# szy4017/DeepSense6G_TII

Hardware: AMD Instinct MI355X
Metric: training samples/sec (5-frame seq, bs=12 per GPU) (higher is better)
Workload: dtype f32; 1 GPU; BASELINE configs[2]: full camera+LiDAR+radar+GPS fusion, 5x(3+1+2)x256x256 + 2x2 GPS per sample, bs=12 per GPU, sigmoid focal loss, AdamW, train-mode BN, dropout 0.1; global_batch=12, seq_len=5, parallelism=dp1, ema=False, launch=eager, optimizer=AdamW after backward

## Files before the change

deepsense6g_tii_amd/csrc/igemm.hip:

```cpp
#include "common.h"
#include "gemm_plan.h"
#include <vector>

extern int g_ds6g_attn_fused128;
extern int g_ds6g_attn_merged_sum;
extern int g_ds6g_attn_percu;
extern int g_ds6g_attn_handover;
extern int g_wino_kb64;

#ifndef IGEMM_STAGES_FD
#define IGEMM_STAGES_FD 3
#endif
#ifndef IGEMM_STAGES_W
#define IGEMM_STAGES_W 2
#endif

GCLK_STORAGE(g_igemm_clk, g_igemm_wg, ds6g_igemm_clocks_read)

namespace {

enum { MODE_FWD = 0, MODE_DGRAD = 1, MODE_WGRAD = 2 };

struct IgemmParams {
    const float* a_src;
    const float* b_src;
    float* out;
    int N, H, W, C;
    int Ho, Wo, K;
    int R, S, stride, pad;
    int Mg, Ng, Kg;
    const float* bias;
    const float* residual;
    const float* mask_src;
    int relu;
    int accumulate;
    uint32_t drop_thr;
    float drop_scale;
    uint64_t seed;
    uint64_t seed_off;
    const uint64_t* salt;
    int k_per_split;
    size_t split_stride;
    int tiles_n;
    int nclass;
    double prof_flops;
    int wg_rows;
    int is_linear;
    int want_colsum;
    int xcd_splits;
    int h0, hstep, Hs, w0, wstep, Ws, r0, rstep, nr, s0, sstep, ns;
    unsigned a_bytes, b_bytes;
    int dbg;
};


template <int MODE, int BM, int BN, int EPI, int BK, int BF, int FAST>
__global__ __launch_bounds__(256) void igemm_kernel(const IgemmParams pin) {
    IgemmParams p = pin;
    if (EPI && p.drop_thr && p.salt) p.seed_off += *p.salt;
    GCLK_DECL(g_igemm_wg);
    if (MODE == MODE_DGRAD && pin.nclass > 1) {
        const int ph = blockIdx.y >> 1, pw = blockIdx.y & 1;
        p.h0 = ph;
        p.w0 = pw;
        p.r0 = (ph + p.pad) & 1;
        p.nr = p.r0 < p.R ? (p.R - p.r0 + 1) / 2 : 0;
        p.s0 = (pw + p.pad) & 1;
        p.ns = p.s0 < p.S ? (p.S - p.s0 + 1) / 2 : 0;
        p.Kg = p.nr * p.ns * p.K;
        if (p.ns == 0) p.ns = 1;
        if (p.Kg == 0 && p.accumulate) return;
    }
    constexpr int CH = BK / 4;
    constexpr int RPB = 16 / CH;
    constexpr int KH = BK / 2;
    constexpr int TM = BM / 64;
    constexpr int TN = BN / 64;
    constexpr int A_LD = BM * CH / 256;
    constexpr int B_LD = BN * CH / 256;
    constexpr bool A_KMAJOR = (MODE == MODE_WGRAD);
    constexpr bool B_KMAJOR = (MODE != MODE_FWD);
    __shared__ __attribute__((aligned(16))) float As0[BM * BK];
    __shared__ __attribute__((aligned(16))) float As1[BM * BK];
    __shared__ __attribute__((aligned(16))) float Bs0[BN * BK];
    __shared__ __attribute__((aligned(16))) float Bs1[BN * BK];
    constexpr int NS = (MODE == MODE_WGRAD) ? IGEMM_STAGES_W : (BK == 32 ? 2 : IGEMM_STAGES_FD);
    static_assert(NS >= 2 && NS <= 4, "2..4 LDS stages");
    __shared__ __attribute__((aligned(16))) float As2[NS >= 3 ? BM * BK : 4];
    __shared__ __attribute__((aligned(16))) float Bs2[NS >= 3 ? BN * BK : 4];
    __shared__ __attribute__((aligned(16))) float As3[NS >= 4 ? BM * BK : 4];
    __shared__ __attribute__((aligned(16))) float Bs3[NS >= 4 ? BN * BK : 4];

    const int tid = threadIdx.x;
    const int lane = tid & 63;
    const int wave = __builtin_amdgcn_readfirstlane(tid >> 6);
    const int wm = wave >> 1, wn = wave & 1;
    int wg, split = blockIdx.z;
    if (MODE == MODE_WGRAD && p.xcd_splits) {
        const int nwg = gridDim.x * gridDim.z, orig = blockIdx.x + gridDim.x * blockIdx.z;
        const int q = nwg >> 3, r = nwg & 7, xcd = orig & 7;
        const int lin = (xcd < r ? xcd * (q + 1) : r * (q + 1) + (xcd - r) * q) + (orig >> 3);
        split = lin / (int)gridDim.x;
        wg = lin - split * (int)gridDim.x;
    } else {
        const int nwg = gridDim.x, orig = blockIdx.x;
        const int q = nwg >> 3, r = nwg & 7, xcd = orig & 7;
        wg = (xcd < r ? xcd * (q + 1) : r * (q + 1) + (xcd - r) * q) + (orig >> 3);
    }
    const int tile_m = wg / p.tiles_n;
    const int tile_n = wg - tile_m * p.tiles_n;
    const int m0 = tile_m * BM, n0 = tile_n * BN;
    const int kbegin = (MODE == MODE_WGRAD) ? split * p.k_per_split : 0;
    const int kend = (MODE == MODE_WGRAD) ? min(p.Kg, kbegin + p.k_per_split) : p.Kg;
    const int nk = (kend - kbegin + BK - 1) / BK;

    const i32x4 a_rsrc = make_srd(p.a_src, p.a_bytes);
    const i32x4 b_rsrc = make_srd(p.b_src, p.b_bytes);

    unsigned a_base[A_LD];
    int a_y[A_LD], a_x[A_LD];
    int a_c[A_LD], a_r[A_LD], a_s[A_LD], a_k[A_LD];
    bool a_ok[A_LD];
#pragma unroll
    for (int i = 0; i < A_LD; ++i) {
        const int idx = tid + i * 256;
        if (MODE == MODE_FWD || MODE == MODE_DGRAD) {
            const int row = idx / CH;
            const int m = m0 + row;
            a_ok[i] = m < p.Mg;
            const int mm = a_ok[i] ? m : 0;
            const int cin = (MODE == MODE_FWD) ? p.C : p.K;
            const int kg = ((idx % CH) ^ ((row / RPB) & (CH - 1))) * 4;
            a_k[i] = kg;
            const int tap = kg / cin;
            a_c[i] = kg - tap * cin;
            const int nsx = (MODE == MODE_DGRAD) ? p.ns : p.S;
            a_r[i] = tap / nsx;
            a_s[i] = tap - a_r[i] * nsx;
            if (MODE == MODE_FWD) {
                int ow, t, oh, n;
                fast_divmod(mm, p.Wo, t, ow);
                fast_divmod(t, p.Ho, n, oh);
                a_y[i] = oh * p.stride - p.pad;
                a_x[i] = ow * p.stride - p.pad;
                a_base[i] = (unsigned)n * (unsigned)(p.H * p.W * p.C);
            } else {
                int ww, t, hh, n;
                fast_divmod(mm, p.Ws, t, ww);
                fast_divmod(t, p.Hs, n, hh);
                a_y[i] = p.h0 + hh * p.hstep + p.pad;
                a_x[i] = p.w0 + ww * p.wstep + p.pad;
                a_base[i] = (unsigned)n * (unsigned)(p.Ho * p.Wo * p.K);
            }
        } else {
            const int mc = idx % (BM / 4);
            a_ok[i] = (m0 + mc * 4) < p.Mg;
            a_k[i] = kbegin + idx / (BM / 4);
            a_base[i] = (unsigned)(m0 + mc * 4);
            a_y[i] = a_x[i] = a_c[i] = a_r[i] = a_s[i] = 0;
        }
    }
    unsigned b_base[B_LD];
    int b_r[B_LD], b_s[B_LD];
    int b_k[B_LD];
    int b_o[B_LD], b_t[B_LD];
    int b_n[B_LD];
    bool b_ok[B_LD];
#pragma unroll
    for (int i = 0; i < B_LD; ++i) {
        const int idx = tid + i * 256;
        b_r[i] = b_s[i] = b_o[i] = b_t[i] = b_n[i] = 0;
        if (MODE == MODE_FWD) {
            const int row = idx / CH;
            b_ok[i] = (n0 + row) < p.Ng;
            b_k[i] = ((idx % CH) ^ ((row / RPB) & (CH - 1))) * 4;
            b_base[i] = (unsigned)(n0 + row) * (unsigned)p.Kg;
        } else if (MODE == MODE_DGRAD) {
            b_ok[i] = (n0 + (idx % (BN / 4)) * 4) < p.Ng;
            const int kg = idx / (BN / 4);
            b_k[i] = kg;
            const int tap = kg / p.K;
            b_o[i] = kg - tap * p.K;
            b_t[i] = tap / p.ns;
            b_n[i] = tap - b_t[i] * p.ns;
            b_base[i] = (unsigned)(n0 + (idx % (BN / 4)) * 4);
        } else {
            const int ncol = n0 + (idx % (BN / 4)) * 4;
            b_ok[i] = ncol < p.Ng;
            const int nn = b_ok[i] ? ncol : 0;
            const int tap = nn / p.C;
            b_r[i] = tap / p.S;
            b_s[i] = tap - b_r[i] * p.S;
            b_base[i] = (unsigned)(nn - tap * p.C);
            const int pix = kbegin + idx / (BN / 4);
            b_k[i] = pix;
            const int pp = pix < p.Kg ? pix : 0;
            b_o[i] = pp % p.Wo;
            const int t = pp / p.Wo;
            b_t[i] = t % p.Ho;
            b_n[i] = t / p.Ho;
        }
    }

    [[maybe_unused]] int u_c0 = 0, u_r = 0, u_s = 0;
    [[maybe_unused]] unsigned u_kb = 0;
    [[maybe_unused]] int u_kpos = kbegin, u_n = 0, u_oh = 0, u_ow = 0;
    [[maybe_unused]] unsigned a_vo[A_LD], b_vo[B_LD];
    [[maybe_unused]] int a_kr[A_LD], b_kr[B_LD], b_ihl[B_LD], b_iwl[B_LD];
    [[maybe_unused]] i32x4 b_rsrc_f = b_rsrc;
    auto retap = [&]() {
#pragma unroll
        for (int i = 0; i < A_LD; ++i) {
            if (MODE == MODE_FWD) {
                const int ih = a_y[i] + u_r, iw = a_x[i] + u_s;
                const bool ok = a_ok[i] && (unsigned)ih < (unsigned)p.H && (unsigned)iw < (unsigned)p.W;
                a_vo[i] = ok ? (a_base[i] + (unsigned)((ih * p.W + iw) * p.C + a_c[i])) * 4u : OOB_OFF;
            } else if (MODE == MODE_DGRAD) {
                const int th = a_y[i] - (p.r0 + u_r * p.rstep), tw = a_x[i] - (p.s0 + u_s * p.sstep);
                int oh = th, ow = tw;
                bool okk = th >= 0 && tw >= 0;
                if (p.stride == 2) {
                    oh = th >> 1;
                    ow = tw >> 1;
                    okk = okk && !((th | tw) & 1);
                } else if (p.stride != 1) {
                    oh = th / p.stride;
                    ow = tw / p.stride;
                    okk = okk && (oh * p.stride == th) && (ow * p.stride == tw);
                }
                const bool ok = a_ok[i] && okk && oh < p.Ho && ow < p.Wo;
                a_vo[i] = ok ? (a_base[i] + (unsigned)((oh * p.Wo + ow) * p.K + a_c[i])) * 4u : OOB_OFF;
            }
        }
    };
    if (FAST) {
        if (MODE == MODE_FWD) {
            retap();
#pragma unroll
            for (int i = 0; i < B_LD; ++i) b_vo[i] = b_ok[i] ? (b_base[i] + (unsigned)b_k[i]) * 4u : OOB_OFF;
        } else if (MODE == MODE_DGRAD) {
            retap();
#pragma unroll
            for (int i = 0; i < B_LD; ++i)
                b_vo[i] = b_ok[i] ? (b_base[i] + (unsigned)(b_o[i] * (p.R * p.S) * p.C)) * 4u : OOB_OFF;
        } else {
            if (p.wg_rows == 0) {
                u_ow = kbegin % p.Wo;
                const int t = kbegin / p.Wo;
                u_oh = t % p.Ho;
                u_n = t / p.Ho;
            } else {
                const int t = kbegin / p.Wo;
                u_oh = t % p.Ho;
                u_n = t / p.Ho;
            }
            const int shift = (p.pad * p.W + p.pad) * p.C;
            b_rsrc_f = make_srd(p.b_src - shift, p.b_bytes + (unsigned)shift * 4u);
#pragma unroll
            for (int i = 0; i < A_LD; ++i) {
                a_kr[i] = (tid + i * 256) / (BM / 4);
                a_vo[i] = (a_base[i] + (unsigned)(a_kr[i] * p.K)) * 4u;
            }
#pragma unroll
            for (int i = 0; i < B_LD; ++i) {
                b_kr[i] = (tid + i * 256) / (BN / 4);
                const int dl_oh = p.wg_rows == 0 ? 0 : b_kr[i] / p.Wo;
                const int dl_ow = p.wg_rows == 0 ? b_kr[i] : b_kr[i] % p.Wo;
                b_ihl[i] = dl_oh * p.stride - p.pad + b_r[i];
                b_iwl[i] = dl_ow * p.stride - p.pad + b_s[i];
                b_vo[i] = (unsigned)((int)b_base[i] + (b_ihl[i] * p.W + b_iwl[i]) * p.C + shift) * 4u;
            }
        }
    }

    auto issue_tiles = [&](float* Ad, float* Bd) {
        if (FAST) {
            if (MODE == MODE_FWD || MODE == MODE_DGRAD) {
                const unsigned sa = (unsigned)u_c0 * 4u;
                unsigned sb;
                if (MODE == MODE_FWD) {
                    sb = u_kb;
                } else {
                    const int tapw = (p.r0 + u_r * p.rstep) * p.S + p.s0 + u_s * p.sstep;
                    sb = (unsigned)((u_c0 * (p.R * p.S) + tapw) * p.C) * 4u;
                }
#pragma unroll
                for (int i = 0; i < A_LD; ++i)
                    dma16(a_rsrc, lds_addr(Ad) + (unsigned)(i * 256 + wave * 64) * 16u, (p.dbg & 32) ? OOB_OFF : a_vo[i], sa);
#pragma unroll
                for (int i = 0; i < B_LD; ++i)
                    dma16(b_rsrc, lds_addr(Bd) + (unsigned)(i * 256 + wave * 64) * 16u, (p.dbg & 32) ? OOB_OFF : b_vo[i], sb);
                u_kb += BK * 4;
                u_c0 += BK;
                if (u_c0 == ((MODE == MODE_FWD) ? p.C : p.K)) {
                    u_c0 = 0;
                    if (++u_s == ((MODE == MODE_FWD) ? p.S : p.ns)) { u_s = 0; ++u_r; }
                    retap();
                }
            } else {
                const int rows_left = kend - u_kpos;
                const unsigned sa = (unsigned)(u_kpos * p.K) * 4u;
                const int ihu = u_oh * p.stride, iwu = u_ow * p.stride;
                const unsigned sb = (unsigned)(((u_n * p.H + ihu) * p.W + iwu) * p.C) * 4u;
#pragma unroll
                for (int i = 0; i < A_LD; ++i) {
                    const bool ok = a_ok[i] && a_kr[i] < rows_left && !(p.dbg & 32);
                    dma16(a_rsrc, lds_addr(Ad) + (unsigned)(i * 256 + wave * 64) * 16u, ok ? a_vo[i] : OOB_OFF, sa);
                }
#pragma unroll
                for (int i = 0; i < B_LD; ++i) {
                    const bool ok = b_ok[i] && b_kr[i] < rows_left && (unsigned)(ihu + b_ihl[i]) < (unsigned)p.H &&
                                    (unsigned)(iwu + b_iwl[i]) < (unsigned)p.W && !(p.dbg & 32);
                    dma16(b_rsrc_f, lds_addr(Bd) + (unsigned)(i * 256 + wave * 64) * 16u, ok ? b_vo[i] : OOB_OFF, sb);
                }
                u_kpos += BK;
                if (p.wg_rows == 0) {
                    u_ow += BK;
                    if (u_ow >= p.Wo) {
                        u_ow = 0;
                        if (++u_oh == p.Ho) { u_oh = 0; ++u_n; }
                    }
                } else {
                    u_oh += p.wg_rows;
                    if (u_oh >= p.Ho) { u_oh = 0; ++u_n; }
                }
            }
            return;
        }
#pragma unroll
        for (int i = 0; i < A_LD; ++i) {
            unsigned off;
            bool ok = a_ok[i] && a_k[i] < kend;
            if (MODE == MODE_FWD) {
                const int ih = a_y[i] + a_r[i], iw = a_x[i] + a_s[i];
                ok = ok && ih >= 0 && ih < p.H && iw >= 0 && iw < p.W;
                off = a_base[i] + (unsigned)((ih * p.W + iw) * p.C + a_c[i]);
            } else if (MODE == MODE_DGRAD) {
                const int th = a_y[i] - (p.r0 + a_r[i] * p.rstep), tw = a_x[i] - (p.s0 + a_s[i] * p.sstep);
                int oh = th, ow = tw;
                bool okk = th >= 0 && tw >= 0;
                if (p.stride == 2) {
                    oh = th >> 1;
                    ow = tw >> 1;
                    okk = okk && !((th | tw) & 1);
                } else if (p.stride != 1) {
                    oh = th / p.stride;
                    ow = tw / p.stride;
                    okk = okk && (oh * p.stride == th) && (ow * p.stride == tw);
                }
                ok = ok && okk && oh < p.Ho && ow < p.Wo;
                off = a_base[i] + (unsigned)((oh * p.Wo + ow) * p.K + a_c[i]);
            } else {
                off = a_base[i] + (unsigned)a_k[i] * (unsigned)p.K;
            }
            if (p.dbg & 32) ok = false;
            dma16(a_rsrc, lds_addr(Ad) + (unsigned)(i * 256 + wave * 64) * 16u, ok ? off * 4u : OOB_OFF, 0u);
            a_k[i] += BK;
            if (MODE != MODE_WGRAD) {
                const int cin = (MODE == MODE_FWD) ? p.C : p.K;
                a_c[i] += BK;
                const int nsx = (MODE == MODE_DGRAD) ? p.ns : p.S;
                while (a_c[i] >= cin) {
                    a_c[i] -= cin;
                    if (++a_s[i] == nsx) { a_s[i] = 0; ++a_r[i]; }
                }
            }
        }
#pragma unroll
        for (int i = 0; i < B_LD; ++i) {
            unsigned off;
            bool ok = b_ok[i] && b_k[i] < kend;
            if (MODE == MODE_FWD) {
                off = b_base[i] + (unsigned)b_k[i];
            } else if (MODE == MODE_DGRAD) {
                const int tap = (p.r0 + b_t[i] * p.rstep) * p.S + p.s0 + b_n[i] * p.sstep;
                off = b_base[i] + (unsigned)((b_o[i] * (p.R * p.S) + tap) * p.C);
                b_o[i] += BK;
                while (b_o[i] >= p.K) {
                    b_o[i] -= p.K;
                    if (++b_n[i] == p.ns) { b_n[i] = 0; ++b_t[i]; }
                }
            } else {
                const int ih = b_t[i] * p.stride - p.pad + b_r[i];
                const int iw = b_o[i] * p.stride - p.pad + b_s[i];
                ok = ok && ih >= 0 && ih < p.H && iw >= 0 && iw < p.W;
                off = b_base[i] + (unsigned)(((b_n[i] * p.H + ih) * p.W + iw) * p.C);
                b_o[i] += BK;
                while (b_o[i] >= p.Wo) {
                    b_o[i] -= p.Wo;
                    if (++b_t[i] == p.Ho) { b_t[i] = 0; ++b_n[i]; }
                }
            }
            if (p.dbg & 32) ok = false;
            dma16(b_rsrc, lds_addr(Bd) + (unsigned)(i * 256 + wave * 64) * 16u, ok ? off * 4u : OOB_OFF, 0u);
            b_k[i] += BK;
        }
    };

    f32x16 acc[TM][TN];
#pragma unroll
    for (int i = 0; i < TM; ++i)
#pragma unroll
        for (int j = 0; j < TN; ++j)
#pragma unroll
            for (int r = 0; r < 16; ++r) acc[i][j][r] = 0.f;

    const int a_row = wm * (BM / 2) + (lane & 31);
    const int b_row = wn * (BN / 2) + (lane & 31);
    const int khalf = lane >> 5;
    const int swz = ((lane & 31) / RPB) & (CH - 1);

    float csum = 0.f;
    const bool do_csum = (MODE == MODE_WGRAD) && p.want_colsum && tile_n == 0 && tid < BM;
    auto k_step = [&](const float* Ac, const float* Bc, float* An, float* Bn, int rem) {
        if (NS >= 3) {
            if (NS >= 4 && rem >= 2) asm volatile("s_waitcnt vmcnt(%0)" ::"n"(2 * (A_LD + B_LD)) : "memory");
            else if (rem >= 1) asm volatile("s_waitcnt vmcnt(%0)" ::"n"(A_LD + B_LD) : "memory");
            else asm volatile("s_waitcnt vmcnt(0)" ::: "memory");
            GCLK(g_igemm_clk, 4);
            if (!(p.dbg & 4)) __syncthreads();
            GCLK(g_igemm_clk, 5);
        }
        if (rem >= NS - 1 && !(p.dbg & 1)) issue_tiles(An, Bn);
        GCLK(g_igemm_clk, 2);
        if (MODE == MODE_WGRAD && do_csum) {
#pragma unroll
            for (int k = 0; k < BK; ++k) csum += Ac[k * BM + tid];
        }
        float af[TM][KH], bf[TN][KH];
#pragma unroll
        for (int i = 0; i < TM; ++i) {
            if (A_KMAJOR) {
#pragma unroll
                for (int kk = 0; kk < KH; ++kk) af[i][kk] = Ac[(khalf * KH + kk) * BM + a_row + i * 32];
            } else {
                const float* rp = &Ac[(a_row + i * 32) * BK];
#pragma unroll
                for (int c = 0; c < CH / 2; ++c) {
                    const f32x4 v = *reinterpret_cast<const f32x4*>(rp + (((khalf * (CH / 2) + c) ^ swz) << 2));
#pragma unroll
                    for (int e = 0; e < 4; ++e) af[i][4 * c + e] = v[e];
                }
            }
        }
#pragma unroll
        for (int j = 0; j < TN; ++j) {
            if (B_KMAJOR) {
#pragma unroll
                for (int kk = 0; kk < KH; ++kk) bf[j][kk] = Bc[(khalf * KH + kk) * BN + b_row + j * 32];
            } else {
                const float* rp = &Bc[(b_row + j * 32) * BK];
#pragma unroll
                for (int c = 0; c < CH / 2; ++c) {
                    const f32x4 v = *reinterpret_cast<const f32x4*>(rp + (((khalf * (CH / 2) + c) ^ swz) << 2));
#pragma unroll
                    for (int e = 0; e < 4; ++e) bf[j][4 * c + e] = v[e];
                }
            }
        }
        __builtin_amdgcn_sched_barrier(0);
        if (BF) {
            static_assert(!BF || BK % 16 == 0, "bf16 k-tiles are multiples of 16");
#pragma unroll
            for (int q = 0; q < BK / 16; ++q) {
                if (BF == 3) {
                    bf16x8 ah[TM], am[TM], al3[TM], bh[TN], bm[TN], bl3[TN];
#pragma unroll
                    for (int i = 0; i < TM; ++i) split3_bf16x8(&af[i][8 * q], ah[i], am[i], al3[i]);
#pragma unroll
                    for (int j = 0; j < TN; ++j) split3_bf16x8(&bf[j][8 * q], bh[j], bm[j], bl3[j]);
#pragma unroll
                    for (int i = 0; i < TM; ++i)
#pragma unroll
                        for (int j = 0; j < TN; ++j)
                            acc[i][j] = mfma_x6(ah[i], am[i], al3[i], bh[j], bm[j], bl3[j], acc[i][j]);
                    continue;
                }
                bf16x8 a8[TM], b8[TN], al[TM], bl[TN];
#pragma unroll
                for (int i = 0; i < TM; ++i) {
                    if (BF == 2) split_bf16x8(&af[i][8 * q], a8[i], al[i]);
                    else {
#pragma unroll
                        for (int e = 0; e < 8; ++e) a8[i][e] = (__bf16)af[i][8 * q + e];
                    }
                }
#pragma unroll
                for (int j = 0; j < TN; ++j) {
                    if (BF == 2) split_bf16x8(&bf[j][8 * q], b8[j], bl[j]);
                    else {
#pragma unroll
                        for (int e = 0; e < 8; ++e) b8[j][e] = (__bf16)bf[j][8 * q + e];
                    }
                }
                if (BF == 2) {
#pragma unroll
                    for (int i = 0; i < TM; ++i)
#pragma unroll
                        for (int j = 0; j < TN; ++j)
                            acc[i][j] = __builtin_amdgcn_mfma_f32_32x32x16_bf16(al[i], b8[j], acc[i][j], 0, 0, 0);
#pragma unroll
                    for (int i = 0; i < TM; ++i)
#pragma unroll
                        for (int j = 0; j < TN; ++j)
                            acc[i][j] = __builtin_amdgcn_mfma_f32_32x32x16_bf16(a8[i], bl[j], acc[i][j], 0, 0, 0);
                }
#pragma unroll
                for (int i = 0; i < TM; ++i)
#pragma unroll
                    for (int j = 0; j < TN; ++j)
                        acc[i][j] = __builtin_amdgcn_mfma_f32_32x32x16_bf16(a8[i], b8[j], acc[i][j], 0, 0, 0);
            }
        } else {
#pragma unroll
            for (int kk = 0; kk < BK / 2; ++kk) {
#pragma unroll
                for (int i = 0; i < TM; ++i)
#pragma unroll
                    for (int j = 0; j < TN; ++j)
                        acc[i][j] = __builtin_amdgcn_mfma_f32_32x32x2f32(af[i][kk], bf[j][kk], acc[i][j], 0, 0, 0);
            }
        }
        __builtin_amdgcn_sched_barrier(0);
        GCLK(g_igemm_clk, 3);
        GCLK_COUNT(g_igemm_clk, 15);
        if (NS == 2) {
            asm volatile("s_waitcnt vmcnt(0)" ::: "memory");
            GCLK(g_igemm_clk, 4);
            if (!(p.dbg & 4)) __syncthreads();
            GCLK(g_igemm_clk, 5);
        }
    };

    float* const Ast[4] = {As0, As1, As2, As3};
    float* const Bst[4] = {Bs0, Bs1, Bs2, Bs3};
    [[maybe_unused]] float bias_pre[TN];
    if (EPI) {
#pragma unroll
        for (int j = 0; j < TN; ++j) {
            const int col = n0 + wn * (BN / 2) + j * 32 + (lane & 31);
            bias_pre[j] = (p.bias && col < p.Ng) ? p.bias[col] : 0.f;
        }
    }
    GCLK(g_igemm_clk, 0);
#pragma unroll
    for (int u = 0; u < NS - 1; ++u)
        if (u < nk && !(p.dbg & 16)) issue_tiles(Ast[u], Bst[u]);
    if (NS == 2) {
        asm volatile("s_waitcnt vmcnt(0)" ::: "memory");
        __syncthreads();
    }
    GCLK(g_igemm_clk, 1);
    for (int kt0 = 0; kt0 < nk; kt0 += NS) {
#pragma unroll
        for (int u = 0; u < NS; ++u) {
            const int kt = kt0 + u;
            if (kt < nk) k_step(Ast[u], Bst[u], Ast[(u + NS - 1) % NS], Bst[(u + NS - 1) % NS], nk - 1 - kt);
        }
    }

    float* outp = p.out + ((MODE == MODE_WGRAD) ? (size_t)split * p.split_stride : (size_t)0);
    if (MODE == MODE_WGRAD && do_csum && m0 + tid < p.Mg) outp[(size_t)p.Mg * p.Ng + m0 + tid] = csum;
    if (EPI == 0) {
        const auto o_rsrc = __builtin_amdgcn_make_buffer_rsrc(outp, 0, (unsigned)p.Mg * (unsigned)p.Ng * 4u, 0x00020000);
        const unsigned rowbytes = (unsigned)p.Ng * 4u;
#pragma unroll
        for (int i = 0; i < TM; ++i) {
#pragma unroll
            for (int j = 0; j < TN; ++j) {
                const int col = n0 + wn * (BN / 2) + j * 32 + (lane & 31);
                const int row0 = m0 + wm * (BM / 2) + i * 32 + 4 * khalf;
                const unsigned base = (col < p.Ng && !((p.dbg & 8) && (i | j)))
                                          ? (unsigned)row0 * rowbytes + (unsigned)col * 4u
                                          : OOB_OFF;
#pragma unroll
                for (int r = 0; r < 16; ++r) {
                    const unsigned off = base + (unsigned)((r & 3) + 8 * (r >> 2)) * rowbytes;
                    float v = acc[i][j][r];
                    if (MODE != MODE_WGRAD && p.accumulate)
                        v += __uint_as_float(__builtin_amdgcn_raw_buffer_load_b32(o_rsrc, off, 0, 0));
                    __builtin_amdgcn_raw_buffer_store_b32(__float_as_uint(v), o_rsrc, off, 0, 0);
                }
            }
        }
        GCLK(g_igemm_clk, 6);
        GCLK_END(g_igemm_clk, g_igemm_wg);
        return;
    }
    if (!(MODE == MODE_DGRAD && p.hstep != 1)) {
        const unsigned nbytes = (unsigned)p.Mg * (unsigned)p.Ng * 4u;
        const auto o_rsrc = __builtin_amdgcn_make_buffer_rsrc(outp, 0, nbytes, 0x00020000);
        const auto m_rsrc = __builtin_amdgcn_make_buffer_rsrc(const_cast<float*>(p.mask_src ? p.mask_src : outp), 0, nbytes, 0x00020000);
        const auto r_rsrc = __builtin_amdgcn_make_buffer_rsrc(const_cast<float*>(p.residual ? p.residual : outp), 0, nbytes, 0x00020000);
        const unsigned rowbytes = (unsigned)p.Ng * 4u;
#pragma unroll
        for (int i = 0; i < TM; ++i) {
#pragma unroll
            for (int j = 0; j < TN; ++j) {
                const int col = n0 + wn * (BN / 2) + j * 32 + (lane & 31);
                const int row0 = m0 + wm * (BM / 2) + i * 32 + 4 * khalf;
                const bool cok = col < p.Ng;
                const float bias = bias_pre[j];
                const unsigned base = cok ? (unsigned)row0 * rowbytes + (unsigned)col * 4u : OOB_OFF;
                const unsigned e0 = (unsigned)row0 * (unsigned)p.Ng + (unsigned)col;
#pragma unroll
                for (int r = 0; r < 16; ++r) {
                    const unsigned dr = (unsigned)((r & 3) + 8 * (r >> 2));
                    const unsigned off = base + dr * rowbytes;
                    float v = acc[i][j][r] + bias;
                    if (p.relu == 1) v = fmaxf(v, 0.f);
                    if (p.mask_src) v = (__uint_as_float(__builtin_amdgcn_raw_buffer_load_b32(m_rsrc, off, 0, 0)) > 0.f) ? v : 0.f;
                    if (p.drop_thr)
                        v = ds6g_keep(p.seed, p.seed_off + (uint64_t)(e0 + dr * (unsigned)p.Ng), p.drop_thr) ? v * p.drop_scale : 0.f;
                    if (p.residual) v += __uint_as_float(__builtin_amdgcn_raw_buffer_load_b32(r_rsrc, off, 0, 0));
                    if (p.accumulate) v += __uint_as_float(__builtin_amdgcn_raw_buffer_load_b32(o_rsrc, off, 0, 0));
                    if (p.relu == 2) v = fmaxf(v, 0.f);
                    __builtin_amdgcn_raw_buffer_store_b32(__float_as_uint(v), o_rsrc, off, 0, 0);
                }
            }
        }
        GCLK(g_igemm_clk, 6);
        GCLK_END(g_igemm_clk, g_igemm_wg);
        return;
    }
#pragma unroll
    for (int i = 0; i < TM; ++i) {
#pragma unroll
        for (int j = 0; j < TN; ++j) {
            const int col = n0 + wn * (BN / 2) + j * 32 + (lane & 31);
            if (col >= p.Ng) continue;
#pragma unroll
            for (int r = 0; r < 16; ++r) {
                const int row = m0 + wm * (BM / 2) + i * 32 + (r & 3) + 8 * (r >> 2) + 4 * khalf;
                if (row >= p.Mg) continue;
                const int ww = row % p.Ws;
                const int t = row / p.Ws;
                const int hh = t % p.Hs;
                const size_t orow = ((size_t)(t / p.Hs) * p.H + p.h0 + hh * p.hstep) * p.W + p.w0 + ww * p.wstep;
                const size_t o = orow * p.Ng + col;
                float v = acc[i][j][r];
                if (p.accumulate) v += outp[o];
                outp[o] = v;
            }
        }
    }
    GCLK(g_igemm_clk, 6);
    GCLK_END(g_igemm_clk, g_igemm_wg);
}

constexpr int RED_COLS = 16, RED_LANES = 16;
__global__ __launch_bounds__(256) void splitk_reduce_kernel(const float* __restrict__ part, float* __restrict__ out,
                                                            long n4, float* __restrict__ out_b, long m4, int splits,
                                                            size_t stride, int accumulate, int accumulate_b) {
    __shared__ f32x4 red[RED_LANES][RED_COLS];
    const int col = threadIdx.x & (RED_COLS - 1), sl = threadIdx.x / RED_COLS;
    const long i = (long)blockIdx.x * RED_COLS + col;
    f32x4 s = {0.f, 0.f, 0.f, 0.f};
    if (i < n4 + m4)
        for (int k = sl; k < splits; k += RED_LANES) s += *reinterpret_cast<const f32x4*>(part + (size_t)k * stride + i * 4);
    red[sl][col] = s;
    __syncthreads();
    if (sl != 0 || i >= n4 + m4) return;
#pragma unroll
    for (int l = 1; l < RED_LANES; ++l) s += red[l][col];
    const bool is_b = i >= n4;
    f32x4* o = is_b ? reinterpret_cast<f32x4*>(out_b + (i - n4) * 4) : reinterpret_cast<f32x4*>(out + i * 4);
    if (is_b ? accumulate_b : accumulate) s += *o;
    *o = s;
}

static_assert(GEMM_ERR_ARG == DS6G_ERR_ARG && GEMM_ERR_WORKSPACE == DS6G_ERR_WORKSPACE && GEMM_OOB == OOB_OFF, "gemm_plan.h");

int g_last_variant = -1;

struct ProfRec { int variant; double flops; hipEvent_t e0, e1; };
std::vector<ProfRec>* g_prof = nullptr;
size_t g_prof_cap = 0;

GemmKnobs g_knobs;
GemmKnobs igemm_knobs() {
    static const bool env_read = [] {
        gemm_env("DS6G_WGRAD_TARGET_LIN", &g_knobs.wgrad_target_lin);
        gemm_env("DS6G_WGRAD_TARGET_CONV", &g_knobs.wgrad_target_conv);
        gemm_env("DS6G_WGRAD_XCD", &g_knobs.wgrad_xcd);
        return true;
    }();
    (void)env_read;
    GemmKnobs kn = g_knobs;
    kn.operand_mode = g_ds6g_bf16;
    return kn;
}

}

void* ds6g_prof_open(int variant, double flops, hipStream_t st) {
    if (!g_prof || g_prof->size() >= g_prof_cap) return nullptr;
    g_prof->push_back(ProfRec{});
    ProfRec* rec = &g_prof->back();
    rec->variant = variant;
    rec->flops = flops;
    (void)hipEventCreate(&rec->e0);
    (void)hipEventCreate(&rec->e1);
    (void)hipEventRecord(rec->e0, st);
    return rec;
}
void ds6g_prof_close(void* rec, hipStream_t st) {
    if (rec) (void)hipEventRecord(static_cast<ProfRec*>(rec)->e1, st);
}

int ds6g_internal_splitk_reduce(const float* ws, float* dw, long n4, float* dbias, long m4, int splits, size_t stride,
                                int accumulate, int accumulate_b, hipStream_t st) {
    hipLaunchKernelGGL(splitk_reduce_kernel, dim3(cdiv(n4 + m4, RED_COLS)), dim3(256), 0, st, ws, dw, n4, dbias, m4, splits,
                       stride, accumulate, accumulate_b);
    DS6G_LAUNCH_CHECK();
    return DS6G_OK;
}

GemmKnobs ds6g_internal_bgemm_knobs();

namespace {

int plan_params(const GemmProblem& q, GemmPlan& pl, IgemmParams& p) {
    if (const int rc = gemm_plan_params(q, igemm_knobs(), pl, p)) return rc;
    p.is_linear = q.op >= DS6G_GEMM_LINEAR_FWD && q.op <= DS6G_GEMM_LINEAR_WGRAD;
    if (pl.nclass > 1) p.prof_flops = 2.0 * p.Mg * p.Ng * (double)(p.R * p.S) * p.K;
    p.dbg = g_knobs.dbg;
    return DS6G_OK;
}

template <int MODE, int CODE>
void launch_igemm(const IgemmParams& p, const GemmPlan& pl, hipStream_t st) {
    constexpr int BF = CODE % 4, KW = CODE / 4 % 3, EPI = CODE / 12 % 2, TILE = CODE / 24;
    constexpr int BM = TILE == 2 ? 64 : 128, BN = TILE == 0 ? 128 : 64;
    if constexpr (!(MODE == MODE_WGRAD && KW == 2))
        hipLaunchKernelGGL((igemm_kernel<MODE, BM, BN, EPI, KW == 2 ? 32 : 16, BF, KW != 0>), dim3(pl.grid_x, pl.grid_y, pl.grid_z),
                           dim3(256), 0, st, p);
}

int run_igemm(const IgemmParams& p, const GemmPlan& pl, float* dw, float* dbias, int accumulate, hipStream_t st) {
    void* rec = ds6g_prof_open(pl.variant, p.prof_flops > 0 ? p.prof_flops : 2.0 * p.Mg * p.Ng * p.Kg, st);
    const int code = ((pl.tile * 2 + pl.epilogue) * 3 + (pl.bk == 32 ? 2 : pl.walk)) * 4 + pl.operand_mode;
    const auto codes = std::make_integer_sequence<int, 3 * 2 * 3 * 4>{};
    if (pl.mode == MODE_FWD) gemm_dispatch(code, [&](auto c) { launch_igemm<MODE_FWD, decltype(c)::value>(p, pl, st); }, codes);
    else if (pl.mode == MODE_DGRAD) gemm_dispatch(code, [&](auto c) { launch_igemm<MODE_DGRAD, decltype(c)::value>(p, pl, st); }, codes);
    else gemm_dispatch(code, [&](auto c) { launch_igemm<MODE_WGRAD, decltype(c)::value>(p, pl, st); }, codes);
    ds6g_prof_close(rec, st);
    g_last_variant = pl.variant;
    DS6G_LAUNCH_CHECK();
    if (!pl.reduce) return DS6G_OK;
    return ds6g_internal_splitk_reduce(p.out, dw, (long)pl.Mg * pl.Ng / 4, dbias, pl.want_colsum ? pl.Mg / 4 : 0, pl.splits,
                                       pl.slab_elems, accumulate, accumulate, st);
}

constexpr int F32 = DS6G_GEMM_F32;

}

extern "C" {

int ds6g_last_igemm_variant(void) { return g_last_variant; }

int ds6g_profile_begin(int max_records) {
    if (max_records <= 0) return DS6G_ERR_ARG;
    if (!g_prof) g_prof = new std::vector<ProfRec>();
    for (auto& r : *g_prof) { (void)hipEventDestroy(r.e0); (void)hipEventDestroy(r.e1); }
    g_prof->clear();
    g_prof->reserve((size_t)max_records);
    g_prof_cap = (size_t)max_records;
    return DS6G_OK;
}

int ds6g_profile_end(int* variants, double* flops, float* ms, int cap) {
    if (!g_prof) return 0;
    int n = 0;
    for (auto& r : *g_prof) {
        (void)hipEventSynchronize(r.e1);
        float t = 0.f;
        (void)hipEventElapsedTime(&t, r.e0, r.e1);
        if (n < cap && variants && flops && ms) { variants[n] = r.variant; flops[n] = r.flops; ms[n] = t; ++n; }
        (void)hipEventDestroy(r.e0);
        (void)hipEventDestroy(r.e1);
    }
    g_prof->clear();
    g_prof_cap = 0;
    return n;
}

int ds6g_set_debug_flags(int flags) {
    g_knobs.dbg = flags & 0xbf;
    g_ds6g_attn_handover = (flags & 0x01000000) ? 0 : 1;
    g_ds6g_attn_fused128 = (flags & 0x04000000) ? 0 : 1;
    g_ds6g_attn_merged_sum = (flags & 0x08000000) ? 0 : 1;
    g_ds6g_attn_percu = (flags >> 20) & 0xf;
    g_wino_kb64 = (flags & 0x02000000) ? 1 : 0;
    g_knobs.bf16_bk32 = (flags & 0x10000000) ? 0 : 1;
    g_knobs.f32_bk32 = (flags & 0x20000000) ? 1 : ((flags & 0x40000000) ? 0 : 2);
    g_knobs.wgrad_tile = (flags & 0x40) ? 2 : 1;
    if ((flags >> 8) & 0xfff) g_knobs.min_blocks = (flags >> 8) & 0xfff;
    return 0;
}

int ds6g_gemm_plan(int family, int op, int N, int H, int W, int C, int K, int R, int S, int stride, int pad, int flags,
                   size_t ws_bytes, struct ds6g_gemm_plan* plan) {
    const GemmProblem q = {family, op, N, H, W, C, K, R, S, stride, pad, (flags & DS6G_GEMM_EPILOGUE) != 0,
                           (flags & DS6G_GEMM_OUT16) != 0, (flags & DS6G_GEMM_ACCUMULATE) != 0, (flags & DS6G_GEMM_DBIAS) != 0, ws_bytes};
    return gemm_plan(q, family == DS6G_GEMM_H16 ? ds6g_internal_bgemm_knobs() : igemm_knobs(), plan);
}

int ds6g_conv2d_fwd(const float* x, const float* w, float* y, int N, int H, int W, int C, int K, int R,
                    int S, int stride, int pad, void* stream) {
    DS6G_ENTER();
    DS6G_CHECK_ARG(x && w && y);
    const GemmProblem q = {F32, DS6G_GEMM_CONV_FWD, N, H, W, C, K, R, S, stride, pad, 0, 0, 0, 0, 0};
    GemmPlan pl; IgemmParams p;
    if (const int rc = plan_params(q, pl, p)) return rc;
    p.a_src = x; p.b_src = w; p.out = y;
    return run_igemm(p, pl, nullptr, nullptr, 0, (hipStream_t)stream);
}

int ds6g_conv2d_dgrad(const float* dy, const float* w, float* dx, int N, int H, int W, int C, int K, int R,
                      int S, int stride, int pad, int accumulate, void* stream) {
    DS6G_ENTER();
    DS6G_CHECK_ARG(dy && w && dx);
    const GemmProblem q = {F32, DS6G_GEMM_CONV_DGRAD, N, H, W, C, K, R, S, stride, pad, 0, 0, accumulate, 0, 0};
    GemmPlan pl; IgemmParams p;
    if (const int rc = plan_params(q, pl, p)) return rc;
    p.a_src = dy; p.b_src = w; p.out = dx;
    return run_igemm(p, pl, nullptr, nullptr, 0, (hipStream_t)stream);
}

int ds6g_conv2d_wgrad(const float* x, const float* dy, float* dw, int N, int H, int W, int C, int K, int R,
                      int S, int stride, int pad, int accumulate, float* ws, size_t ws_bytes, void* stream) {
    DS6G_ENTER();
    DS6G_CHECK_ARG(x && dy && dw);
    const GemmProblem q = {F32, DS6G_GEMM_CONV_WGRAD, N, H, W, C, K, R, S, stride, pad, 0, 0, accumulate, 0, ws_bytes};
    GemmPlan pl; IgemmParams p;
    if (const int rc = plan_params(q, pl, p)) return rc;
    DS6G_CHECK_ARG(ws || !pl.reduce);
    p.a_src = dy; p.b_src = x; p.out = pl.reduce ? ws : dw;
    return run_igemm(p, pl, dw, nullptr, accumulate, (hipStream_t)stream);
}

int ds6g_conv2d_bias_act_fwd(const float* x, const float* w, const float* bias, const float* residual, float* y, int N,
                             int H, int W, int C, int K, int R, int S, int stride, int pad, int relu, void* stream) {
    DS6G_ENTER();
    DS6G_CHECK_ARG(x && w && y && relu >= 0 && relu <= 2);
    const GemmProblem q = {F32, DS6G_GEMM_CONV_BIAS_ACT_FWD, N, H, W, C, K, R, S, stride, pad, bias || relu || residual, 0, 0, 0, 0};
    GemmPlan pl; IgemmParams p;
    if (const int rc = plan_params(q, pl, p)) return rc;
    p.a_src = x; p.b_src = w; p.out = y; p.bias = bias; p.residual = residual; p.relu = relu;
    return run_igemm(p, pl, nullptr, nullptr, 0, (hipStream_t)stream);
}

int ds6g_linear_fwd(const float* x, const float* w, const float* bias, float* y, int M, int N, int K, int relu,
                    const float* residual, float drop_p, uint64_t seed, uint64_t seed_off, void* stream) {
    DS6G_ENTER();
    DS6G_CHECK_ARG(x && w && y && drop_p >= 0.f && drop_p < 1.f);
    const uint32_t drop_thr = ds6g_drop_threshold(drop_p);
    const GemmProblem q = {F32, DS6G_GEMM_LINEAR_FWD, 1, 1, M, K, N, 1, 1, 1, 0, bias || relu || drop_thr || residual, 0, 0, 0, 0};
    GemmPlan pl; IgemmParams p;
    if (const int rc = plan_params(q, pl, p)) return rc;
    p.a_src = x; p.b_src = w; p.out = y; p.bias = bias; p.relu = relu; p.residual = residual;
    p.drop_thr = drop_thr;
    p.drop_scale = 1.f / (1.f - drop_p);
    p.seed = seed; p.seed_off = seed_off; p.salt = g_ds6g_salt;
    return run_igemm(p, pl, nullptr, nullptr, 0, (hipStream_t)stream);
}

int ds6g_linear_dgrad(const float* dy, const float* w, float* dx, int M, int N, int K, const float* mask_src,
                      int accumulate, void* stream) {
    DS6G_ENTER();
    DS6G_CHECK_ARG(dy && w && dx);
    const GemmProblem q = {F32, DS6G_GEMM_LINEAR_DGRAD, 1, 1, M, K, N, 1, 1, 1, 0, mask_src != nullptr, 0, accumulate, 0, 0};
    GemmPlan pl; IgemmParams p;
    if (const int rc = plan_params(q, pl, p)) return rc;
    p.a_src = dy; p.b_src = w; p.out = dx; p.mask_src = mask_src;
    return run_igemm(p, pl, nullptr, nullptr, 0, (hipStream_t)stream);
}

int ds6g_linear_wgrad(const float* x, const float* dy, float* dw, float* dbias, int M, int N, int K, int accumulate,
                      float* ws, size_t ws_bytes, void* stream) {
    DS6G_ENTER();
    DS6G_CHECK_ARG(x && dy && dw);
    const GemmProblem q = {F32, DS6G_GEMM_LINEAR_WGRAD, 1, 1, M, K, N, 1, 1, 1, 0, 0, 0, accumulate, dbias != nullptr, ws_bytes};
    GemmPlan pl; IgemmParams p;
    if (const int rc = plan_params(q, pl, p)) return rc;
    DS6G_CHECK_ARG(ws || !pl.reduce);
    p.a_src = dy; p.b_src = x; p.out = pl.reduce ? ws : dw;
    return run_igemm(p, pl, dw, dbias, accumulate, (hipStream_t)stream);
}

}
```

Baseline: 185.8 samples/s.

## Software-pipeline igemm epilogue loads and add occupancy launch bounds

Restructures the igemm epilogues so the residual, mask and accumulate loads for the next output tile are issued while the current tile is being computed and stored, using double buffers and scheduling barriers. Adds min-waves launch bounds derived from the LDS footprint to steer register allocation toward higher occupancy. Replaces per-element div/mod in the strided dgrad scatter with one fast_divmod per row block plus a cheap reciprocal-based divmod, and routes those writes through buffer loads and stores. It also stops instantiating WGRAD kernels with the epilogue variant. The risk is extra register pressure from the prefetch buffers, or spills forced by the tighter launch bounds.

```diff
diff --git a/deepsense6g_tii_amd/csrc/igemm.hip b/deepsense6g_tii_amd/csrc/igemm.hip
--- a/deepsense6g_tii_amd/csrc/igemm.hip
+++ b/deepsense6g_tii_amd/csrc/igemm.hip
@@ -20,6 +20,13 @@
 namespace {
 
 enum { MODE_FWD = 0, MODE_DGRAD = 1, MODE_WGRAD = 2 };
+
+__device__ __forceinline__ void small_divmod(int m, int d, int& q, int& r) {
+    q = (int)((float)m * __builtin_amdgcn_rcpf((float)d));
+    r = m - q * d;
+    if (r < 0) { --q; r += d; }
+    else if (r >= d) { ++q; r -= d; }
+}
 
 struct IgemmParams {
     const float* a_src;
@@ -54,8 +61,14 @@
 };
 
 
+constexpr int igemm_min_waves(int MODE, int BM, int BN, int EPI, int BK, int BF, int FAST) {
+    if (MODE == MODE_WGRAD) return 1;
+    const int lds = (BK == 32 ? 2 : IGEMM_STAGES_FD) * (BM + BN) * BK * 4, w = 160 * 1024 / lds < 8 ? 160 * 1024 / lds : 8;
+    return BF == 3 && (BM == 64 || (BN == 128 && MODE == MODE_DGRAD && EPI && !FAST)) ? w - 1 : w;
+}
+
 template <int MODE, int BM, int BN, int EPI, int BK, int BF, int FAST>
-__global__ __launch_bounds__(256) void igemm_kernel(const IgemmParams pin) {
+__global__ __launch_bounds__(256, igemm_min_waves(MODE, BM, BN, EPI, BK, BF, FAST)) void igemm_kernel(const IgemmParams pin) {
     IgemmParams p = pin;
     if (EPI && p.drop_thr && p.salt) p.seed_off += *p.salt;
     GCLK_DECL(g_igemm_wg);
@@ -561,26 +574,50 @@
 
     float* outp = p.out + ((MODE == MODE_WGRAD) ? (size_t)split * p.split_stride : (size_t)0);
     if (MODE == MODE_WGRAD && do_csum && m0 + tid < p.Mg) outp[(size_t)p.Mg * p.Ng + m0 + tid] = csum;
+    constexpr int NT = TM * TN;
+    const auto ld16 = [](const __amdgpu_buffer_rsrc_t rs, unsigned base, unsigned rowbytes, float (&dst)[16]) {
+        asm volatile("" : "+v"(base));
+#pragma unroll
+        for (int r = 0; r < 16; ++r)
+            dst[r] = __uint_as_float(__builtin_amdgcn_raw_buffer_load_b32(rs, base + (unsigned)((r & 3) + 8 * (r >> 2)) * rowbytes, 0, 0));
+    };
+    const auto st16 = [](const __amdgpu_buffer_rsrc_t rs, unsigned base, unsigned rowbytes, const float (&v)[16]) {
+        asm volatile("" : "+v"(base));
+#pragma unroll
+        for (int r = 0; r < 16; ++r)
+            __builtin_amdgcn_raw_buffer_store_b32(__float_as_uint(v[r]), rs, base + (unsigned)((r & 3) + 8 * (r >> 2)) * rowbytes, 0, 0);
+    };
     if (EPI == 0) {
         const auto o_rsrc = __builtin_amdgcn_make_buffer_rsrc(outp, 0, (unsigned)p.Mg * (unsigned)p.Ng * 4u, 0x00020000);
         const unsigned rowbytes = (unsigned)p.Ng * 4u;
-#pragma unroll
-        for (int i = 0; i < TM; ++i) {
-#pragma unroll
-            for (int j = 0; j < TN; ++j) {
-                const int col = n0 + wn * (BN / 2) + j * 32 + (lane & 31);
-                const int row0 = m0 + wm * (BM / 2) + i * 32 + 4 * khalf;
-                const unsigned base = (col < p.Ng && !((p.dbg & 8) && (i | j)))
-                                          ? (unsigned)row0 * rowbytes + (unsigned)col * 4u
-                                          : OOB_OFF;
-#pragma unroll
-                for (int r = 0; r < 16; ++r) {
-                    const unsigned off = base + (unsigned)((r & 3) + 8 * (r >> 2)) * rowbytes;
-                    float v = acc[i][j][r];
-                    if (MODE != MODE_WGRAD && p.accumulate)
-                        v += __uint_as_float(__builtin_amdgcn_raw_buffer_load_b32(o_rsrc, off, 0, 0));
-                    __builtin_amdgcn_raw_buffer_store_b32(__float_as_uint(v), o_rsrc, off, 0, 0);
-                }
+        const auto base_of = [&](int t) -> unsigned {
+            const int i = t / TN, j = t % TN;
+            const int col = n0 + wn * (BN / 2) + j * 32 + (lane & 31);
+            const int row0 = m0 + wm * (BM / 2) + i * 32 + 4 * khalf;
+            return (col < p.Ng && !((p.dbg & 8) && (i | j))) ? (unsigned)row0 * rowbytes + (unsigned)col * 4u : OOB_OFF;
+        };
+        if (MODE != MODE_WGRAD && p.accumulate) {
+            float po[2][16];
+            ld16(o_rsrc, base_of(0), rowbytes, po[0]);
+#pragma unroll
+            for (int t = 0; t < NT; ++t) {
+                const f32x16& a = acc[t / TN][t % TN];
+                float v[16];
+#pragma unroll
+                for (int r = 0; r < 16; ++r) v[r] = a[r] + po[t & 1][r];
+                if (t + 1 < NT) ld16(o_rsrc, base_of(t + 1), rowbytes, po[(t + 1) & 1]);
+                st16(o_rsrc, base_of(t), rowbytes, v);
+                __builtin_amdgcn_sched_barrier(0);
+            }
+        } else {
+#pragma unroll
+            for (int t = 0; t < NT; ++t) {
+                const f32x16& a = acc[t / TN][t % TN];
+                float v[16];
+#pragma unroll
+                for (int r = 0; r < 16; ++r) v[r] = a[r];
+                st16(o_rsrc, base_of(t), rowbytes, v);
+                __builtin_amdgcn_sched_barrier(0);
             }
         }
         GCLK(g_igemm_clk, 6);
@@ -593,54 +630,118 @@
         const auto m_rsrc = __builtin_amdgcn_make_buffer_rsrc(const_cast<float*>(p.mask_src ? p.mask_src : outp), 0, nbytes, 0x00020000);
         const auto r_rsrc = __builtin_amdgcn_make_buffer_rsrc(const_cast<float*>(p.residual ? p.residual : outp), 0, nbytes, 0x00020000);
         const unsigned rowbytes = (unsigned)p.Ng * 4u;
-#pragma unroll
-        for (int i = 0; i < TM; ++i) {
-#pragma unroll
-            for (int j = 0; j < TN; ++j) {
+        const bool has_m = p.mask_src != nullptr, has_r = p.residual != nullptr, has_o = p.accumulate != 0;
+        float pa[2][16], po[2][16];
+        const auto base_of = [&](int t) -> unsigned {
+            const int i = t / TN, j = t % TN;
+            const int col = n0 + wn * (BN / 2) + j * 32 + (lane & 31);
+            const int row0 = m0 + wm * (BM / 2) + i * 32 + 4 * khalf;
+            return col < p.Ng ? (unsigned)row0 * rowbytes + (unsigned)col * 4u : OOB_OFF;
+        };
+        const auto issue = [&](int t) {
+            const int b = t & 1;
+            if (has_m) ld16(m_rsrc, base_of(t), rowbytes, pa[b]);
+            else if (has_r) ld16(r_rsrc, base_of(t), rowbytes, pa[b]);
+            if (has_o) ld16(o_rsrc, base_of(t), rowbytes, po[b]);
+        };
+#pragma unroll
+        for (int j = 0; j < TN; ++j) asm volatile("" : "+v"(bias_pre[j]));
+        issue(0);
+#pragma unroll
+        for (int t = 0; t < NT; ++t) {
+            const int i = t / TN, j = t % TN, b = t & 1;
+            unsigned keeps = 0u;
+            if (p.drop_thr) {
                 const int col = n0 + wn * (BN / 2) + j * 32 + (lane & 31);
                 const int row0 = m0 + wm * (BM / 2) + i * 32 + 4 * khalf;
-                const bool cok = col < p.Ng;
-                const float bias = bias_pre[j];
-                const unsigned base = cok ? (unsigned)row0 * rowbytes + (unsigned)col * 4u : OOB_OFF;
                 const unsigned e0 = (unsigned)row0 * (unsigned)p.Ng + (unsigned)col;
 #pragma unroll
                 for (int r = 0; r < 16; ++r) {
                     const unsigned dr = (unsigned)((r & 3) + 8 * (r >> 2));
-                    const unsigned off = base + dr * rowbytes;
-                    float v = acc[i][j][r] + bias;
-                    if (p.relu == 1) v = fmaxf(v, 0.f);
-                    if (p.mask_src) v = (__uint_as_float(__builtin_amdgcn_raw_buffer_load_b32(m_rsrc, off, 0, 0)) > 0.f) ? v : 0.f;
-                    if (p.drop_thr)
-                        v = ds6g_keep(p.seed, p.seed_off + (uint64_t)(e0 + dr * (unsigned)p.Ng), p.drop_thr) ? v * p.drop_scale : 0.f;
-                    if (p.residual) v += __uint_as_float(__builtin_amdgcn_raw_buffer_load_b32(r_rsrc, off, 0, 0));
-                    if (p.accumulate) v += __uint_as_float(__builtin_amdgcn_raw_buffer_load_b32(o_rsrc, off, 0, 0));
-                    if (p.relu == 2) v = fmaxf(v, 0.f);
-                    __builtin_amdgcn_raw_buffer_store_b32(__float_as_uint(v), o_rsrc, off, 0, 0);
-                }
-            }
+                    keeps |= (ds6g_keep(p.seed, p.seed_off + (uint64_t)(e0 + dr * (unsigned)p.Ng), p.drop_thr) ? 1u : 0u) << r;
+                }
+            }
+            const float bias = bias_pre[j];
+            const f32x16& a = acc[i][j];
+            float v[16];
+#pragma unroll
+            for (int r = 0; r < 16; ++r) v[r] = a[r] + bias;
+            if (p.relu == 1) {
+#pragma unroll
+                for (int r = 0; r < 16; ++r) v[r] = fmaxf(v[r], 0.f);
+            }
+            if (has_m) {
+#pragma unroll
+                for (int r = 0; r < 16; ++r) {
+                    float m = pa[b][r];
+                    asm volatile("" : "+v"(m));
+                    v[r] = (m > 0.f) ? v[r] : 0.f;
+                }
+            }
+            if (p.drop_thr) {
+#pragma unroll
+                for (int r = 0; r < 16; ++r) v[r] = ((keeps >> r) & 1u) ? v[r] * p.drop_scale : 0.f;
+            }
+            if (has_r) {
+                if (has_m) ld16(r_rsrc, base_of(t), rowbytes, pa[b]);
+#pragma unroll
+                for (int r = 0; r < 16; ++r) v[r] += pa[b][r];
+            }
+            if (has_o) {
+#pragma unroll
+                for (int r = 0; r < 16; ++r) v[r] += po[b][r];
+            }
+            if (p.relu == 2) {
+#pragma unroll
+                for (int r = 0; r < 16; ++r) v[r] = fmaxf(v[r], 0.f);
+            }
+            if (t + 1 < NT) issue(t + 1);
+            st16(o_rsrc, base_of(t), rowbytes, v);
+            __builtin_amdgcn_sched_barrier(0);
         }
         GCLK(g_igemm_clk, 6);
         GCLK_END(g_igemm_clk, g_igemm_wg);
         return;
     }
-#pragma unroll
-    for (int i = 0; i < TM; ++i) {
-#pragma unroll
-        for (int j = 0; j < TN; ++j) {
-            const int col = n0 + wn * (BN / 2) + j * 32 + (lane & 31);
-            if (col >= p.Ng) continue;
+    {
+        const auto o_rsrc = __builtin_amdgcn_make_buffer_rsrc(
+            outp, 0, (unsigned)p.N * (unsigned)p.H * (unsigned)p.W * (unsigned)p.Ng * 4u, 0x00020000);
+#pragma unroll
+        for (int i = 0; i < TM; ++i) {
+            unsigned rowoff[16];
+            const int row0 = m0 + wm * (BM / 2) + i * 32 + 4 * khalf;
+            int ww0, t0, hh0, n0i;
+            fast_divmod(row0, p.Ws, t0, ww0);
+            fast_divmod(t0, p.Hs, n0i, hh0);
 #pragma unroll
             for (int r = 0; r < 16; ++r) {
-                const int row = m0 + wm * (BM / 2) + i * 32 + (r & 3) + 8 * (r >> 2) + 4 * khalf;
-                if (row >= p.Mg) continue;
-                const int ww = row % p.Ws;
-                const int t = row / p.Ws;
-                const int hh = t % p.Hs;
-                const size_t orow = ((size_t)(t / p.Hs) * p.H + p.h0 + hh * p.hstep) * p.W + p.w0 + ww * p.wstep;
-                const size_t o = orow * p.Ng + col;
-                float v = acc[i][j][r];
-                if (p.accumulate) v += outp[o];
-                outp[o] = v;
+                const int dr = (r & 3) + 8 * (r >> 2);
+                int ww, tq, hh, nq;
+                small_divmod(ww0 + dr, p.Ws, tq, ww);
+                small_divmod(hh0 + tq, p.Hs, nq, hh);
+                const unsigned orow = (unsigned)(((n0i + nq) * p.H + p.h0 + hh * p.hstep) * p.W + p.w0 + ww * p.wstep);
+                rowoff[r] = row0 + dr < p.Mg ? orow * (unsigned)p.Ng * 4u : OOB_OFF;
+            }
+#pragma unroll
+            for (int j = 0; j < TN; ++j) {
+                const int col = n0 + wn * (BN / 2) + j * 32 + (lane & 31);
+                const unsigned cb = col < p.Ng ? (unsigned)col * 4u : OOB_OFF;
+                unsigned off[16];
+#pragma unroll
+                for (int r = 0; r < 16; ++r) off[r] = (rowoff[r] | cb) >= OOB_OFF ? OOB_OFF : rowoff[r] + cb;
+                const f32x16& a = acc[i][j];
+                float v[16];
+#pragma unroll
+                for (int r = 0; r < 16; ++r) v[r] = a[r];
+                if (p.accumulate) {
+                    float po[16];
+#pragma unroll
+                    for (int r = 0; r < 16; ++r) po[r] = __uint_as_float(__builtin_amdgcn_raw_buffer_load_b32(o_rsrc, off[r], 0, 0));
+#pragma unroll
+                    for (int r = 0; r < 16; ++r) v[r] += po[r];
+                }
+#pragma unroll
+                for (int r = 0; r < 16; ++r) __builtin_amdgcn_raw_buffer_store_b32(__float_as_uint(v[r]), o_rsrc, off[r], 0, 0);
             }
         }
     }
@@ -732,7 +833,7 @@
 void launch_igemm(const IgemmParams& p, const GemmPlan& pl, hipStream_t st) {
     constexpr int BF = CODE % 4, KW = CODE / 4 % 3, EPI = CODE / 12 % 2, TILE = CODE / 24;
     constexpr int BM = TILE == 2 ? 64 : 128, BN = TILE == 0 ? 128 : 64;
-    if constexpr (!(MODE == MODE_WGRAD && KW == 2))
+    if constexpr (!(MODE == MODE_WGRAD && (KW == 2 || EPI)))
         hipLaunchKernelGGL((igemm_kernel<MODE, BM, BN, EPI, KW == 2 ? 32 : 16, BF, KW != 0>), dim3(pl.grid_x, pl.grid_y, pl.grid_z),
                            dim3(256), 0, st, p);
 }
```

Result: no change. 187.6 samples/s (median of 6 runs) (+1.0%).
